# KIT-MBS/pydca

Measured on AMD Instinct MI355X. Metric: plmDCA L-BFGS iterations/s (L=500 N=50000 q=21), higher is better.
Workload: dtype f32

## Files before the change

pydca_amd/csrc/lbfgs_kernels.h:

```cpp
#pragma once

#include "dca_internal.h"
#include "plm_plan.h"
#include "vec_kernels.h"

namespace {

template <bool DD> struct DotAcc;
template <> struct DotAcc<false> {
    double hi = 0.0;
    static constexpr double lo = 0.0;
    __device__ __forceinline__ void add(double a, double b) { hi += a * b; }
    __device__ __forceinline__ void wave_reduce() { for (int off = 32; off > 0; off >>= 1) hi += __shfl_down(hi, off); }
};
template <> struct DotAcc<true> {
    double hi = 0.0, lo = 0.0;
    __device__ __forceinline__ void add(double a, double b) { dd_add(hi, lo, __dmul_rn(a, b)); }
    __device__ __forceinline__ void wave_reduce() { dd_wave_reduce(hi, lo); }
};
template <int NV>
__device__ __forceinline__ void dot_block_store(double (*red)[2 * NV], int nv, double* __restrict__ partials, unsigned grid = 0)
{
    __syncthreads();
    if ((int)threadIdx.x < nv) {
// ... 19 lines not shown
            s0.add(av, bv); s1.add(cv, cv); s2.add(av, av);
        },
        { const double av = a[i]; const double bv = b[i]; const double cv = c[i]; s0.add(av, bv); s1.add(cv, cv); s2.add(av, av); })
    s0.wave_reduce(); s1.wave_reduce(); s2.wave_reduce();
    if ((threadIdx.x & 63) == 0) {
        double* r = red[threadIdx.x >> 6];
        r[0] = s0.hi; r[1] = s0.lo; r[2] = s1.hi; r[3] = s1.lo; r[4] = s2.hi; r[5] = s2.lo;
    }
    dot_block_store<3>(red, 3, partials);
}
struct VecPtrs5 { const void* s[5]; const void* y[5]; };
struct DirCoefs { double g; double s[5]; double y[5]; };

struct LbfgsDev { double SY[5][5]; double YY[5][5]; double ys[5]; DirCoefs cf; };
constexpr int kSlotDginit = 30;

__global__ void lbfgs_two_loop_kernel(double* __restrict__ scal, LbfgsDev* __restrict__ st, int e, int endNext, int bound, double gg)
{
    if (threadIdx.x != 0 || blockIdx.x != 0) return;
    constexpr int M = 5;
    const double ys = scal[1], yy = scal[2];
    const double* G5 = scal + 3;
    double Sg[M], Yg[M], alpha[M];
    st->ys[e] = ys;
    for (int k2 = 0; k2 < M; ++k2) {
        Sg[k2] = G5[k2]; Yg[k2] = G5[5 + k2];
        st->SY[e][k2] = G5[10 + k2];
        st->SY[k2][e] = G5[15 + k2];
        st->YY[e][k2] = G5[20 + k2];
        st->YY[k2][e] = G5[20 + k2];
        alpha[k2] = 0.0;
    }
    st->SY[e][e] = ys; st->YY[e][e] = yy;
    DirCoefs cf;
    cf.g = -1.0;
    for (int k2 = 0; k2 < M; ++k2) cf.s[k2] = cf.y[k2] = 0.0;
    int j = endNext;
// ... 50 lines not shown
          const double gv = g[i]; const double sev = sev_; const double yev = yev_;
          acc[0].add(yev, sev); acc[1].add(yev, yev);
          _Pragma("unroll") for (int k = 0; k < 5; ++k) {
              const double sk = k == E ? sev : (double)static_cast<const T*>(P.s[k])[i]; const double yk = k == E ? yev : (double)static_cast<const T*>(P.y[k])[i];
              acc[2 + k].add(sk, gv); acc[7 + k].add(yk, gv); acc[12 + k].add(sev, yk); acc[17 + k].add(yev, sk); acc[22 + k].add(yev, yk);
          } })
    const int lane = threadIdx.x & 63, wv = threadIdx.x >> 6;
#pragma unroll
    for (int v = 0; v < 27; ++v) {
        acc[v].wave_reduce();
        if (lane == 0) { red[wv][2 * v] = acc[v].hi; red[wv][2 * v + 1] = acc[v].lo; }
    }
    dot_block_store<27>(red, 27, partials);
}

template <typename T>
__global__ void vec_compose_kernel(T* __restrict__ d, const T* __restrict__ g, VecPtrs5 P, const DirCoefs* __restrict__ cp, size_t n)
{
    const DirCoefs c = *cp;
    DCA_VEC_LOOP(n, d,
        const Pack<T> pg = ldp(g, iv);
        double v[VEC];
        _Pragma("unroll") for (int u = 0; u < VEC; ++u) v[u] = c.g * (double)pg.v[u];
        _Pragma("unroll") for (int k = 0; k < 5; ++k) {
            const Pack<T> psk = ldp(static_cast<const T*>(P.s[k]), iv); const Pack<T> pyk = ldp(static_cast<const T*>(P.y[k]), iv);
            _Pragma("unroll") for (int u = 0; u < VEC; ++u) v[u] += c.s[k] * (double)psk.v[u] + c.y[k] * (double)pyk.v[u];
        }
        Pack<T> o;
        _Pragma("unroll") for (int u = 0; u < VEC; ++u) o.v[u] = (T)v[u];
        stp(d, iv, o);,
        { double v = c.g * (double)g[i];
          _Pragma("unroll") for (int k = 0; k < 5; ++k)
              v += c.s[k] * (double)static_cast<const T*>(P.s[k])[i] + c.y[k] * (double)static_cast<const T*>(P.y[k])[i];
          d[i] = (T)v; })
}
#undef ldp
#undef stp

__host__ __device__ constexpr int fused_step_ti(int q, int elemBytes) { return kRowBytes / elemBytes / q; }
__host__ __device__ constexpr int fused_step_jc(int q) { return q == 21 ? 4 : 16; }
constexpr int kFusedStepThreads = 512;

template <typename T>
__device__ __forceinline__ T compose_elem(const DirCoefs& c, T gv, const T* sv, const T* yv)
{
    double v = c.g * (double)gv;
#pragma unroll
    for (int k = 0; k < 5; ++k) v += c.s[k] * (double)sv[k] + c.y[k] * (double)yv[k];
    return (T)v;
}

template <typename T, int Q>
__global__ __launch_bounds__(kFusedStepThreads)
void lbfgs_dir_trial_expand_kernel(T* __restrict__ d, T* __restrict__ xt, T* __restrict__ W, const T* __restrict__ x, const T* __restrict__ g,
                                   VecPtrs5 P, const DirCoefs* __restrict__ cp, int L, int Cs, int numJC, int pairBlocks)
// ... 9 lines not shown
    const int tid = threadIdx.x;
    const int padded = (pairBlocks + 63) / 64 * 64;
    if ((int)blockIdx.x >= padded) {
        const size_t e = (size_t)((int)blockIdx.x - padded) * kFusedStepThreads + tid;
        if (e < (size_t)L * Q) {
            T sv[5], yv[5];
#pragma unroll
            for (int k = 0; k < 5; ++k) { sv[k] = static_cast<const T*>(P.s[k])[e]; yv[k] = static_cast<const T*>(P.y[k])[e]; }
            const T dv = compose_elem(c, g[e], sv, yv);
            d[e] = dv;
            const T v = one * dv;
            xt[e] = x[e] + v;
        }
        return;
    }
    const int blk = ((int)blockIdx.x & ~63) | (((int)blockIdx.x & 7) << 3) | (((int)blockIdx.x >> 3) & 7);
    if (blk >= pairBlocks) return;
    const int i0 = (blk / numJC) * TI, j0 = (blk % numJC) * JC;
    const int j1 = min(j0 + JC, L);
    if (j1 <= i0 + 1) return;
    if (tid == 0) {
        int pre = 0;
        for (int ii = 0; ii < TI; ++ii) {
            const int i = i0 + ii, jlo = max(j0, i + 1);
            const int cnt = jlo < j1 ? (j1 - jlo) * Q2 : 0;
            const size_t before = (size_t)L * (L - 1) / 2 - (size_t)(L - i) * (L - i - 1) / 2;
            const size_t lo = cnt ? (size_t)L * Q + (before + (size_t)(jlo - i - 1)) * Q2 : 0;
            sLo[ii] = lo; sCnt[ii] = cnt; sPre[ii] = pre;
            pre += cnt ? (int)((lo + cnt + VEC - 1) / VEC - lo / VEC) : 0;
        }
        sPre[TI] = pre;
    }
    __syncthreads();
    const int total = sPre[TI];
    for (int idx = tid; idx < total; idx += kFusedStepThreads) {
// ... 81 lines not shown
{
    __shared__ double redHi[1024], redLo[1024];
    double hi = 0.0, lo = 0.0;
    for (int b = threadIdx.x; b < nA; b += blockDim.x) dd_add2(hi, lo, A[2 * (size_t)b], A[2 * (size_t)b + 1]);
    for (int b = threadIdx.x; b < nB; b += blockDim.x) dd_add2(hi, lo, B[2 * (size_t)b], B[2 * (size_t)b + 1]);
    dd_block_reduce(hi, lo, redHi, redLo);
    if (threadIdx.x == 0) out[0] = hi + lo;
}

template <typename T>
__global__ __launch_bounds__(kVecThreads)
void vec_dot3_fx_kernel(const T* __restrict__ a, const T* __restrict__ b, const T* __restrict__ c, size_t n, double* __restrict__ partials,
                        const double* __restrict__ fxParts, int nFxParts, double* __restrict__ fxChunks)
{
    if (blockIdx.x >= (unsigned)kVecBlocks) {
        __shared__ double redHi[256], redLo[256];
        const int blk = (int)blockIdx.x - kVecBlocks;
        const int chunk = (nFxParts + kSumStageBlocks - 1) / kSumStageBlocks;
        const int lo_ = blk * chunk, hi_ = min(nFxParts, lo_ + chunk);
        double hi = 0.0, lo = 0.0;
        for (int p = lo_ + threadIdx.x; p < hi_; p += blockDim.x) dd_add2(hi, lo, fxParts[2 * (size_t)p], fxParts[2 * (size_t)p + 1]);
        dd_block_reduce(hi, lo, redHi, redLo);
        if (threadIdx.x == 0) { fxChunks[2 * blk] = hi; fxChunks[2 * blk + 1] = lo; }
        return;
    }
    __shared__ double red[kVecThreads / 64][6];
    DotAcc<sizeof(T) == 8> s0, s1, s2;
    DCA_VEC_LOOP_G(n, a, kVecBlocks,
        const Pack<T> pa = ldp_at(a + head_, iv); const Pack<T> pb = ldp_at(b + head_, iv); const Pack<T> pc = ldp_at(c + head_, iv);
        _Pragma("unroll") for (int k = 0; k < VEC; ++k) {
            const double av = pa.v[k]; const double bv = pb.v[k]; const double cv = pc.v[k];
            s0.add(av, bv); s1.add(cv, cv); s2.add(av, av);
        },
        { const double av = a[i]; const double bv = b[i]; const double cv = c[i]; s0.add(av, bv); s1.add(cv, cv); s2.add(av, av); })
    s0.wave_reduce(); s1.wave_reduce(); s2.wave_reduce();
    if ((threadIdx.x & 63) == 0) {
        double* r = red[threadIdx.x >> 6];
        r[0] = s0.hi; r[1] = s0.lo; r[2] = s1.hi; r[3] = s1.lo; r[4] = s2.hi; r[5] = s2.lo;
    }
    dot_block_store<3>(red, 3, partials, kVecBlocks);
}
__global__ __launch_bounds__(1024)
void vec_final_fx_kernel(const double* __restrict__ partials, int nb, int nk, double* __restrict__ out,
                         const double* __restrict__ A, int nA, const double* __restrict__ B, int nB, double* __restrict__ fxOut)
{
    __shared__ double redHi[1024], redLo[1024];
    const int k = blockIdx.x;
    double hi = 0.0, lo = 0.0;
    if (k < nk) {
        constexpr int NT = 256;
        if ((int)threadIdx.x < NT) {
            for (int b = threadIdx.x; b < nb; b += NT) dd_add2(hi, lo, partials[2 * ((size_t)k * nb + b)], partials[2 * ((size_t)k * nb + b) + 1]);
            redHi[threadIdx.x] = hi;
            redLo[threadIdx.x] = lo;
        }
        __syncthreads();
        for (int st = NT / 2; st > 0; st >>= 1) {
            if ((int)threadIdx.x < st) dd_add2(redHi[threadIdx.x], redLo[threadIdx.x], redHi[threadIdx.x + st], redLo[threadIdx.x + st]);
            __syncthreads();
        }
        if (threadIdx.x == 0) out[k] = redHi[0] + redLo[0];
        return;
    }
    for (int b = threadIdx.x; b < nA; b += blockDim.x) dd_add2(hi, lo, A[2 * (size_t)b], A[2 * (size_t)b + 1]);
    for (int b = threadIdx.x; b < nB; b += blockDim.x) dd_add2(hi, lo, B[2 * (size_t)b], B[2 * (size_t)b + 1]);
    dd_block_reduce(hi, lo, redHi, redLo);
    if (threadIdx.x == 0) fxOut[0] = hi + lo;
}

}
```

pydca_amd/csrc/plm_engine.hip:

```cpp
#include <algorithm>
#include <chrono>
#include <cmath>

#include "dca_internal.h"
#include "more_thuente.h"
#include "vec_kernels.h"
#include "plm_plan.h"
#include "plm_stages.h"
#include "lbfgs_kernels.h"

namespace {

static_assert(kPlanXcds == kNumXcd, "the planner deals strips to this many XCDs");

#ifdef DCA_ROUND_ABLATE
__global__ void round_to_f32_kernel(double* __restrict__ p, size_t n)
{
    for (size_t i = blockIdx.x * (size_t)blockDim.x + threadIdx.x; i < n; i += (size_t)gridDim.x * blockDim.x) p[i] = (double)(float)p[i];
}
inline int round_stage_mask() { const char* e = getenv("DCA_ROUND_F32_STAGES"); return e ? atoi(e) : 0; }
#define DCA_ROUND_STAGE(bit, ptr, count)                                                                             \
    do {                                                                                                             \
        if constexpr (sizeof(T) == 8)                                                                                \
            if (round_stage_mask() & (bit))                                                                          \
// ... 40 lines not shown
    bool lbfgs_alloc = false;
    bool deferFx = false, fxPending = false;
    size_t vlo = 0, vn = 0, Ppad = 0;
    dca_comm_hook comm = nullptr;
    void* comm_user = nullptr;
    int comm_rank = 0, comm_world = 0;

    struct {
        bool begun = false, finished = false;
        int status = 0, k = 1, end = 0, iters = 0, evals = 0, max_iterations = 0, verbose = 0;
        double fx = 0, step = 0, xnorm = 0, gnorm = 0, seconds = 0;
        double last_step = 0;
        double dginit = 0;
        bool dginit_on_device = false;
        bool trial_ready = false;
    } o;

    explicit PlmEngine(dca_ctx* c) : ctx(c), N(c->N), L(c->L), q(c->q), Ls(c->Ls) {}

    template <typename U> int dalloc(U** p, size_t n)
    {
        HIP_TRY(dca_dev_malloc(reinterpret_cast<void**>(p), std::max<size_t>(n, 1) * sizeof(U)));
        return DCA_OK;
    }
    void freeall() { each_buffer([](auto*& p) { dca_dev_free(p); p = nullptr; }); }
    ~PlmEngine() override { freeall(); }

    void weights_changed() override { configured = false; o = decltype(o)(); }

    int configure(double lh, double lJ, int cmode, int chunk_, int warm_, int halo_, int add_reg_) override
// ... 30 lines not shown
        lbfgs_alloc = false;
        o = decltype(o)();

        DCA_TRY(dalloc(&dx, plan.P + kVecPad)); DCA_TRY(dalloc(&dg, plan.P + kVecPad));
        DCA_TRY(dalloc(&dWt, (size_t)plan.Wrows * plan.Cs));
        DCA_TRY(dalloc(&dSR, (size_t)N * plan.Cs));
        DCA_TRY(dalloc(&dR, (size_t)(N + kNC) * plan.Cs));
        HIP_TRY(hipMemsetAsync(dR, 0, (size_t)(N + kNC) * plan.Cs * sizeof(T), ctx->stream));
        DCA_TRY(dalloc(&dG, plan.num_slabs() * plan.slab_elems()));
        DCA_TRY(dalloc(&dw, N));
        DCA_TRY(dalloc(&dXL, (size_t)ceil_div(plan.gUnits, JT) * JT * plan.Npad));
        DCA_TRY(dalloc(&dXT2, (size_t)plan.gUnits * plan.NT));
        DCA_TRY(dalloc(&dPairs, npairs));
        DCA_TRY(dalloc(&dFxPart, 2 * (size_t)plan.nFxPart));
        DCA_TRY(dalloc(&dRegPart, 2 * (size_t)(plan.nRegPart + kSumStageBlocks)));
        DCA_TRY(dalloc(&dVecPart, 2 * 27 * kVecBlocks));
        HIP_TRY(hipMemsetAsync(dRegPart, 0, 2 * (size_t)(plan.nRegPart + kSumStageBlocks) * sizeof(double), ctx->stream));
        HIP_TRY(hipMemsetAsync(dFxPart, 0, 2 * (size_t)plan.nFxPart * sizeof(double), ctx->stream));
        if (sizeof(T) == 8) {
            DCA_TRY(dalloc(&dColPart, 2 * (size_t)kColSumRowBlocks * Lq));
            if (q == 5) DCA_TRY(dalloc(&dColChunk, 2 * (size_t)plan.numScanChunks * Lq));
            DCA_TRY(dalloc(&dColSum, (size_t)Lq));
        }
        if (strips) { DCA_TRY(dalloc(&dGrecv, plan.grecvOff[sWorld])); DCA_TRY(dalloc(&dXsend, plan.xsendOff[sWorld])); DCA_TRY(dalloc(&dXrecv, plan.xrecvOff[sWorld])); }

        HIP_TRY(hipMemsetAsync(dx, 0, (plan.P + kVecPad) * sizeof(T), ctx->stream));
        HIP_TRY(hipMemsetAsync(dg, 0, (plan.P + kVecPad) * sizeof(T), ctx->stream));
        vlo = 0; vn = plan.P; Ppad = plan.P;
        if (strips) {
            native_mode = 4;
            vlo = plan.oLo; vn = plan.oHi - plan.oLo;
// ... 219 lines not shown
                else
                    hipLaunchKernelGGL(plm_colsum_parts_kernel<T>, dim3(ceil_div(LqLoc, 64), kColSumRowBlocks), dim3(256), 0, st, dR, N, plan.Cs, LqLoc, dColPart);
                hipLaunchKernelGGL(plm_colsum_final_kernel, dim3(ceil_div(LqLoc, 256)), dim3(256), 0, st, dColPart, kColSumRowBlocks, LqLoc, dColSum);
            }
            const int nOwned = plan.pairEnd - plan.pairBegin;
            const bool mergeFields = knobs.foldMerge != 0 && !strips && nOwned > 0;
            if (!mergeFields)
            hipLaunchKernelGGL(plm_fold_fields_kernel<T>, dim3(ceil_div(LqLoc, 256)), dim3(256), 0, st, dx + (size_t)plan.cS0 * q, dG, dg + (size_t)plan.cS0 * q,
                               dRegPart + 2 * npairs, LqLoc, q, plan.Cs, (T)lambda_h, add_reg, plan.slab_elems(), foldSlabs, dColSum);
            StripMap sm;
            sm.rank = sRank; sm.world = sWorld; sm.s0 = plan.cS0; sm.s1 = plan.cS1;
            for (int r = 0; r <= sWorld; ++r) sm.site0[r] = plan.siteB[r];
            for (int r = 0; r < sWorld; ++r) { sm.recv[r] = strips && r > sRank ? dGrecv + plan.grecvOff[r] : nullptr; sm.recvCs[r] = strips ? strip_cs(r) : 0; }
            if (strips && !stripEmulate) DCA_TRY(exchange_g());
            const size_t lds = (size_t)kFoldWaves * ((q * q + 3) / 4 * 4) * sizeof(T);
            if (nOwned > 0) {
                const int pairBlocks = ceil_div(nOwned, kFoldWaves);
                FoldFieldsArgs<T> ff{dx + (size_t)plan.cS0 * q, dg + (size_t)plan.cS0 * q, dRegPart + 2 * npairs, LqLoc, (T)lambda_h, dColSum, mergeFields ? pairBlocks : -1};
                hipLaunchKernelGGL(plm_fold_pairs_kernel<T>, dim3((unsigned)(pairBlocks + (mergeFields ? ceil_div(LqLoc, 256) : 0))), dim3(64 * kFoldWaves), lds, st, dx, dG, dg, dPairs,
                                   dRegPart, L, q, plan.Cs, (T)lambda_J, add_reg, plan.slab_elems(), foldSlabs, plan.pairBegin, plan.pairEnd, sm, ff);
            }
        }
        DCA_ROUND_STAGE(16, dg, plan.P);
        fxPending = deferFx;
        if (!deferFx) {
            hipLaunchKernelGGL(dd_sum_chunks_kernel, dim3(kSumStageBlocks), dim3(256), 0, st, dRegPart, plan.nRegPart, dRegPart + 2 * (size_t)plan.nRegPart);
            hipLaunchKernelGGL(dd_sum_final_kernel, dim3(1), dim3(1024), 0, st, dRegPart + 2 * (size_t)plan.nRegPart, kSumStageBlocks, dFxPart, plan.nFxPart, ctx->dScal);
        }
        HIP_TRY(hipGetLastError());
        return DCA_OK;
    }
// ... 176 lines not shown
    }

    int gradient(double* fx_out) override
    {
        o.trial_ready = false;
        DCA_TRY(evaluate_async());
        DCA_TRY(reduce_scalars(0, 1));
        DCA_TRY(gather_vector(dg));
        DCA_TRY(read_scalars(1));
        if (fx_out) *fx_out = ctx->hScal[0];
        return DCA_OK;
    }

    void v_neg(T* d, const T* g) { hipLaunchKernelGGL(vec_neg_kernel<T>, dim3(kVecBlocks), dim3(kVecThreads), 0, ctx->stream, d + vlo, g + vlo, vn); }
    void v_step(T* x, const T* xp, double stp, const T* d) { hipLaunchKernelGGL(vec_step_kernel<T>, dim3(kVecBlocks), dim3(kVecThreads), 0, ctx->stream, x + vlo, xp + vlo, (T)stp, d + vlo, vn); }
    int eval_scalars(double* fx, double* gd, double* xx, double* gg)
    {
        if (fxPending) {
            double* const fxChunks = dRegPart + 2 * (size_t)plan.nRegPart;
            hipLaunchKernelGGL(vec_dot3_fx_kernel<T>, dim3(kVecBlocks + kSumStageBlocks), dim3(kVecThreads), 0, ctx->stream, dg + vlo, dd + vlo, dx + vlo, vn, dVecPart,
                               dRegPart, plan.nRegPart, fxChunks);
            hipLaunchKernelGGL(vec_final_fx_kernel, dim3(3 + 1), dim3(1024), 0, ctx->stream, dVecPart, kVecBlocks, 3, ctx->dScal + 1,
                               fxChunks, kSumStageBlocks, dFxPart, plan.nFxPart, ctx->dScal);
            fxPending = false;
        } else {
            hipLaunchKernelGGL(vec_dot3_kernel<T>, dim3(kVecBlocks), dim3(kVecThreads), 0, ctx->stream, dg + vlo, dd + vlo, dx + vlo, vn, dVecPart);
            hipLaunchKernelGGL(vec_final_kernel, dim3(3), dim3(256), 0, ctx->stream, dVecPart, kVecBlocks, 3, ctx->dScal + 1);
        }
        DCA_TRY(reduce_scalars(0, 4));
        DCA_TRY(read_scalars(kSlotDginit + 1));
        *fx = ctx->hScal[0]; *gd = ctx->hScal[1]; *xx = ctx->hScal[2]; *gg = ctx->hScal[3];
        if (o.dginit_on_device) { o.dginit = ctx->hScal[kSlotDginit]; o.dginit_on_device = false; }
        return DCA_OK;
    }

    int lbfgs_begin(int max_iterations, int verbose) override
    {
// ... 33 lines not shown

    int line_search(double* stp, double* f, double* xx, double* gg, int* rc_hip)
    {
        const MtParams params{1e-4, 0.9, 1e-16, 1e-20, 1e20, 5};
        const bool deferred = o.dginit_on_device;
        bool first = true;
        const int ls = mt_line_search(params, stp, f, &o.dginit, deferred, [&](double t, double* ft, double* dgt) {
            const bool ready = o.trial_ready && first && t == 1.0 && fused_step_ok();
            o.trial_ready = false; first = false;
            if (!ready) {
                v_step(dx, dxp, t, dd);
                DCA_ROUND_STAGE(32, dx, plan.P);
            }
            DCA_TRY(publish_x());
            DCA_TRY(evaluate_async(true, ready));
            return eval_scalars(ft, dgt, xx, gg);
        }, rc_hip);
        if (deferred && ls == LB_INCREASEGRADIENT) o.evals -= 1;
        return ls;
    }

    void lbfgs_end() override { o = decltype(o)(); }
    bool fused_step_ok() const
    {
#ifdef DCA_ROUND_ABLATE
        if (round_stage_mask()) return false;
#endif
        return knobs.fuseStep != 0 && native_mode == 0 && !hook && !comm && !strips && !stripEmulate && vlo == 0 && vn == plan.P &&
               plan.cS0 == 0 && plan.cS1 == L;
    }
    template <int Q> void launch_fused_step(const VecPtrs5& ptrs)
    {
        const int numJC = ceil_div(L, fused_step_jc(Q)), pairBlocks = ceil_div(L, fused_step_ti(Q, (int)sizeof(T))) * numJC;
        const size_t lds = (size_t)fused_step_ti(Q, (int)sizeof(T)) * fused_step_jc(Q) * Q * Q * sizeof(T);
        hipLaunchKernelGGL((lbfgs_dir_trial_expand_kernel<T, Q>), dim3((unsigned)(ceil_div(pairBlocks, 64) * 64 + ceil_div(L * Q, kFusedStepThreads))), dim3(kFusedStepThreads), lds,
                           ctx->stream, dd, dxp, dWt, dx, dg, ptrs, &dLb->cf, L, plan.Cs, numJC, pairBlocks);
    }
    int lbfgs_iterate(int iterations, dca_plm_stats* st) override
    {
        if (!o.begun) { dca_set_error("dca_plm_lbfgs_begin first"); return DCA_ERR_STATE; }
        auto t0 = std::chrono::steady_clock::now();
        constexpr int M = 5;
        for (int it = 0; it < iterations && !o.finished; ++it) {
            std::swap(dx, dxp);
            std::swap(dg, dgp);
// ... 10 lines not shown
            }
            o.xnorm = std::sqrt(xx); o.gnorm = std::sqrt(gg);
            o.iters = o.k;
            o.last_step = o.step;
            if (o.verbose) {
                fprintf(stderr, "Iteration %d:\n", o.k);
                fprintf(stderr, "fx = %f, xnorm = %f, gnorm = %f, step = %f\n\n", o.fx, o.xnorm, o.gnorm, o.step);
            }
            const double xn = std::max(o.xnorm, 1.0);
            if (o.gnorm / xn <= 1e-3) { o.status = 0; o.finished = true; break; }
            if (o.max_iterations != 0 && o.max_iterations < o.k + 1) { o.status = LB_MAXIMUMITERATION; o.finished = true; break; }

            const int e = o.end;
            VecPtrs5 ptrs;
            for (int i = 0; i < M; ++i) { ptrs.s[i] = dS[i] + vlo; ptrs.y[i] = dY[i] + vlo; }
            {
                ScopedKernelClock kc(ctx, "lbfgs_vec");
                auto gram = [&](auto slot) {
                    hipLaunchKernelGGL((vec_diff_gram_kernel<T, decltype(slot)::value>), dim3(kVecBlocks), dim3(kVecThreads), 0, ctx->stream, ptrs, dS[e] + vlo, dY[e] + vlo,
                                       dx + vlo, dxp + vlo, dg + vlo, dgp + vlo, vn, dVecPart);
                };
                switch (e) {
                case 0: gram(std::integral_constant<int, 0>()); break;
                case 1: gram(std::integral_constant<int, 1>()); break;
                case 2: gram(std::integral_constant<int, 2>()); break;
                case 3: gram(std::integral_constant<int, 3>()); break;
                default: gram(std::integral_constant<int, 4>()); break;
                }
                hipLaunchKernelGGL(vec_final_kernel, dim3(27), dim3(256), 0, ctx->stream, dVecPart, kVecBlocks, 27, ctx->dScal + 1);
            }
            DCA_TRY(reduce_scalars(1, 27));
            const int bound = (M <= o.k) ? M : o.k;
            ++o.k;
            o.end = (o.end + 1) % M;
            {
                ScopedKernelClock kc(ctx, "lbfgs_vec");
                hipLaunchKernelGGL(lbfgs_two_loop_kernel, dim3(1), dim3(64), 0, ctx->stream, ctx->dScal, dLb, e, o.end, bound, gg);
                if (fused_step_ok()) {
                    if (q == 21) launch_fused_step<21>(ptrs); else launch_fused_step<5>(ptrs);
                    o.trial_ready = true;
                } else {
                    hipLaunchKernelGGL(vec_compose_kernel<T>, dim3(kVecBlocks), dim3(kVecThreads), 0, ctx->stream, dd + vlo, dg + vlo, ptrs, &dLb->cf, vn);
                    DCA_ROUND_STAGE(64, dd, plan.P);
                }
                o.dginit_on_device = true;
            }
            o.step = 1.0;
        }
        HIP_TRY(hipStreamSynchronize(ctx->stream));
        o.seconds += std::chrono::duration<double>(std::chrono::steady_clock::now() - t0).count();
        if (st) {
            st->status = o.status; st->iterations = o.iters; st->evaluations = o.evals; st->finished = o.finished ? 1 : 0;
// ... 57 lines not shown
```

pydca_amd/csrc/plm_plan.h:

```cpp
#pragma once

#include <algorithm>
#include <cstddef>
#include <cstdlib>
#include <vector>

#include "../../include/dca_hip.h"

namespace {

constexpr int kPlanXcds = 8;
constexpr int kPairQ = 25;
constexpr int kNC = 128;
constexpr int kRowBytes = 512;
constexpr int kScatWavesC = 16;
constexpr int kCanonBlock = 16384;
static_assert(kCanonBlock % kNC == 0, "canonical blocks are whole tiles");
constexpr int kColSumRowBlocks = 64;
constexpr int kSumStageBlocks = 64;
constexpr int kMaxStripRanks = 64;
constexpr size_t kVecPad = 256;

struct PlmShape {
    int N = 0, L = 0, q = 0;
// ... 3 lines not shown
    int carryMode = DCA_CARRY_CHUNKED;
    int stripWorld = 1, stripRank = 0;
    bool strips = false;
};

struct PlmKnobs {
    int scatterRem = -1;
    int scatterSplit = -1;
    int scatterCanon = -1;
    int scatterWaves = -1;
    int plmPairs = -1;
    int scatterMerge = -1;
    int foldMerge = -1;
    int fuseFx = -1;
    int fuseStep = -1;
    bool is_set(int v) const { return v != -1; }
    static PlmKnobs from_env()
    {
        PlmKnobs k;
        auto rd = [](const char* name, int& v) { if (const char* e = getenv(name)) { v = atoi(e); if (v == -1) v = -2; } };
        rd("DCA_SCATTER_REM", k.scatterRem); rd("DCA_SCATTER_SPLIT", k.scatterSplit); rd("DCA_SCATTER_CANON", k.scatterCanon);
        rd("DCA_SCATTER_WAVES", k.scatterWaves); rd("DCA_PLM_PAIRS", k.plmPairs); rd("DCA_SCATTER_MERGE", k.scatterMerge);
        rd("DCA_FOLD_MERGE", k.foldMerge); rd("DCA_PLM_FUSE_FX", k.fuseFx);
        rd("DCA_PLM_FUSE_STEP", k.fuseStep);
        return k;
    }
};

struct PlmKernelShapes {
    int logitsSeqPerWg[3];
    int logitsJT[3];
    static int slot(int q) { return q == 21 ? 1 : q == kPairQ ? 2 : 0; }
};

struct ScatterLaunch {
    unsigned gridX = 0, gridY = 1;
    int N = 0, L = 0, Cs = 0, halo = 0, numChunks = 0, NT = 0, ctBase = 0, numPairs = 0, splitX = 1, numJG = 0, chunksPerSplit = 0;
    size_t slabElems = 0;
    int blockChunks = 0;
// ... 209 lines not shown
```

pydca_amd/csrc/plm_stages.h:

```cpp
#pragma once

#include "dca_internal.h"
#include "plm_plan.h"
#include "vec_kernels.h"

namespace {

#ifdef DCA_FAST_EXP
__device__ __forceinline__ float t_exp(float v) { return __expf(v); }
#else
__device__ __forceinline__ float t_exp(float v) { return expf(v); }
#endif
__device__ __forceinline__ double t_exp(double v) { return exp(v); }
__device__ __forceinline__ float t_log(float v) { return logf(v); }
__device__ __forceinline__ double t_log(double v) { return log(v); }

struct PairIJ { uint16_t i, j; };

template <typename T>
__global__ void plm_expand_kernel(const T* __restrict__ x, T* __restrict__ W, const PairIJ* __restrict__ pairs,
                                  int L, int q, int Cs, int s0, int s1)
{
    extern __shared__ __attribute__((aligned(16))) unsigned char dca_smem[];
    T* tile = reinterpret_cast<T*>(dca_smem);
// ... 633 lines not shown
    T a = G[off];
    for (int sidx = 1; sidx < nsplit; ++sidx) a += G[(size_t)sidx * slabElems + off];
    return a;
}

constexpr int kFoldWaves = 4;
struct StripMap {
    int rank = 0, world = 1, s0 = 0, s1 = 0;
    int site0[kMaxStripRanks + 1];
    const void* recv[kMaxStripRanks];
    int recvCs[kMaxStripRanks];
};
template <typename T>
__device__ __forceinline__ void fold_fields_body(const T* __restrict__ x, const T* __restrict__ G, T* __restrict__ g,
                                                 double* __restrict__ regPart, int Lq, int q, int Cs, T lambdaH, int addReg,
                                                 size_t slabElems, int nsplit, const double* __restrict__ colSum, int blk)
{
    __shared__ double red[256];
    const int c = blk * blockDim.x + threadIdx.x;
    double reg = 0.0;
    if (c < Lq) {
        const T xv = x[c];
        T gv = addReg ? (T)2 * lambdaH * xv : (T)0;
        T s = 0;
        if (colSum) s = (T)colSum[c];
        else for (int b = 0; b < q; ++b) s += slab_sum(G, (size_t)b * Cs + c, slabElems, nsplit);
        g[c] = gv + s;
        if (addReg) reg = (double)lambdaH * (double)xv * (double)xv;
    }
    __shared__ double redLo[256];
    red[threadIdx.x] = reg;
    redLo[threadIdx.x] = 0.0;
    __syncthreads();
    for (int s = blockDim.x / 2; s > 0; s >>= 1) {
        if ((int)threadIdx.x < s) dd_add2(red[threadIdx.x], redLo[threadIdx.x], red[threadIdx.x + s], redLo[threadIdx.x + s]);
        __syncthreads();
    }
    if (threadIdx.x == 0) { regPart[2 * (size_t)blk] = red[0]; regPart[2 * (size_t)blk + 1] = redLo[0]; }
}
template <typename T>
__global__ void plm_fold_fields_kernel(const T* __restrict__ x, const T* __restrict__ G, T* __restrict__ g,
                                       double* __restrict__ regPart, int Lq, int q, int Cs, T lambdaH, int addReg,
                                       size_t slabElems, int nsplit, const double* __restrict__ colSum)
{
    fold_fields_body<T>(x, G, g, regPart, Lq, q, Cs, lambdaH, addReg, slabElems, nsplit, colSum, (int)blockIdx.x);
}
template <typename T> struct FoldFieldsArgs { const T* x; T* g; double* regPart; int Lq; T lambdaH; const double* colSum; int pairBlocks; };
template <typename T>
__global__ __launch_bounds__(64 * kFoldWaves)
void plm_fold_pairs_kernel(const T* __restrict__ x, const T* __restrict__ G, T* __restrict__ g,
                           const PairIJ* __restrict__ pairs, double* __restrict__ regPart,
                           int L, int q, int Cs, T lambdaJ, int addReg, size_t slabElems, int nsplit, int pairBegin, int pairEnd,
                           const StripMap sm, const FoldFieldsArgs<T> ff)
{
    extern __shared__ __attribute__((aligned(16))) unsigned char dca_smem[];
    if (ff.pairBlocks >= 0 && (int)blockIdx.x >= ff.pairBlocks) {
        fold_fields_body<T>(ff.x, G, ff.g, ff.regPart, ff.Lq, q, Cs, ff.lambdaH, addReg, slabElems, nsplit, ff.colSum, (int)blockIdx.x - ff.pairBlocks);
        return;
    }
    const int q2 = q * q;
    const int wave = threadIdx.x >> 6, lane = threadIdx.x & 63;
    T* tile = reinterpret_cast<T*>(dca_smem) + (size_t)wave * ((q2 + 3) / 4 * 4);
    const int p = pairBegin + blockIdx.x * kFoldWaves + wave;
    if (p >= pairEnd) return;
    const int i = pairs[p].i, j = pairs[p].j;
    const int ic = (i - sm.s0) * q;
    for (int t = lane; t < q2; t += 64) {
        const int b = t / q, a = t % q;
        tile[t] = slab_sum(G, (size_t)(j * q + b) * Cs + ic + a, slabElems, nsplit);
    }
    const T* Gj = G;
    size_t jRow = (size_t)i * q, jCs = (size_t)Cs;
// ... 10 lines not shown
    const size_t base = (size_t)L * q + (size_t)p * q2;
    double reg = 0.0, regLo = 0.0;
    for (int t = lane; t < q2; t += 64) {
        const int a = t / q, b = t % q;
        const T xv = x[base + t];
        T gv = addReg ? (T)2 * lambdaJ * xv : (T)0;
        gv += tile[b * q + a];
        gv += slab_sum(Gj, (jRow + a) * jCs + jc + b, slabElems, jSplit);
        g[base + t] = gv;
        if (addReg) dd_add(reg, regLo, (double)lambdaJ * (double)xv * (double)xv);
    }
    dd_wave_reduce(reg, regLo);
    if (lane == 0) { regPart[2 * (size_t)p] = reg; regPart[2 * (size_t)p + 1] = regLo; }
}

}
```

Measured before the change: 61.42.

## Merge eval-scalar dots with L-BFGS gram pass and add tiled pair fold kernel

Adds a kernel that computes the line-search scalars (g·d, x·x, g·g) together with the s/y difference vectors and the 27 gram dots in one pass, so the two-loop update can reuse the gram results instead of rereading all vectors. It also adds an opt-in tiled fold kernel that accumulates pair couplings through LDS tiles instead of per-pair waves, and factors the tile mapping into a shared header. The merged pass removes a full memory sweep and a launch per iteration, at the cost of higher register pressure in the wider fused kernel.

```diff
diff --git a/pydca_amd/csrc/lbfgs_kernels.h b/pydca_amd/csrc/lbfgs_kernels.h
--- a/pydca_amd/csrc/lbfgs_kernels.h
+++ b/pydca_amd/csrc/lbfgs_kernels.h
@@ -2,6 +2,7 @@
 
 #include "dca_internal.h"
 #include "plm_plan.h"
+#include "plm_tiles.h"
 #include "vec_kernels.h"
 
 namespace {
@@ -57,13 +58,14 @@
 
 struct LbfgsDev { double SY[5][5]; double YY[5][5]; double ys[5]; DirCoefs cf; };
 constexpr int kSlotDginit = 30;
-
-__global__ void lbfgs_two_loop_kernel(double* __restrict__ scal, LbfgsDev* __restrict__ st, int e, int endNext, int bound, double gg)
+constexpr int kSlotGram = 32;
+
+__global__ void lbfgs_two_loop_kernel(double* __restrict__ scal, const double* __restrict__ gram, LbfgsDev* __restrict__ st, int e, int endNext, int bound, double gg)
 {
     if (threadIdx.x != 0 || blockIdx.x != 0) return;
     constexpr int M = 5;
-    const double ys = scal[1], yy = scal[2];
-    const double* G5 = scal + 3;
+    const double ys = gram[0], yy = gram[1];
+    const double* G5 = gram + 2;
     double Sg[M], Yg[M], alpha[M];
     st->ys[e] = ys;
     for (int k2 = 0; k2 < M; ++k2) {
@@ -144,6 +146,82 @@
     dot_block_store<27>(red, 27, partials);
 }
 
+__device__ __forceinline__ void fx_chunk_sum(const double* __restrict__ fxParts, int nFxParts, double* __restrict__ fxChunks, int blk)
+{
+    __shared__ double redHi[256], redLo[256];
+    const int chunk = (nFxParts + kSumStageBlocks - 1) / kSumStageBlocks;
+    const int lo_ = blk * chunk, hi_ = min(nFxParts, lo_ + chunk);
+    double hi = 0.0, lo = 0.0;
+    for (int p = lo_ + threadIdx.x; p < hi_; p += blockDim.x) dd_add2(hi, lo, fxParts[2 * (size_t)p], fxParts[2 * (size_t)p + 1]);
+    dd_block_reduce(hi, lo, redHi, redLo);
+    if (threadIdx.x == 0) { fxChunks[2 * blk] = hi; fxChunks[2 * blk + 1] = lo; }
+}
+
+constexpr int kEvalGramDots = 30;
+template <typename T, int E>
+__global__ __launch_bounds__(kVecThreads)
+void vec_eval_gram_kernel(VecPtrs5 P, T* __restrict__ se, T* __restrict__ ye, const T* __restrict__ x, const T* __restrict__ xp,
+                          const T* __restrict__ g, const T* __restrict__ gp, const T* __restrict__ d, size_t n, double* __restrict__ partials,
+                          const double* __restrict__ fxParts, int nFxParts, double* __restrict__ fxChunks)
+{
+    if (blockIdx.x >= (unsigned)kVecBlocks) {
+        fx_chunk_sum(fxParts, nFxParts, fxChunks, (int)blockIdx.x - kVecBlocks);
+        return;
+    }
+    __shared__ double red[kVecThreads / 64][2 * kEvalGramDots];
+    DotAcc<sizeof(T) == 8> ls[3];
+    DotAcc<sizeof(T) == 8> acc[27];
+    DCA_VEC_LOOP_G(n, se, kVecBlocks,
+        const Pack<T> px = ldp(x, iv); const Pack<T> pxp = ldp(xp, iv); const Pack<T> pg = ldp(g, iv); const Pack<T> pgp = ldp(gp, iv);
+        const Pack<T> pd = ldp(d, iv);
+        Pack<T> psk[5]; Pack<T> pyk[5];
+        _Pragma("unroll") for (int k = 0; k < 5; ++k)
+            if (k != E) { psk[k] = ldp(static_cast<const T*>(P.s[k]), iv); pyk[k] = ldp(static_cast<const T*>(P.y[k]), iv); }
+        Pack<T> pse; Pack<T> pye;
+        _Pragma("unroll") for (int u = 0; u < VEC; ++u) {
+            const double gv = pg.v[u]; const double dv = pd.v[u]; const double xv = px.v[u];
+            ls[0].add(gv, dv); ls[1].add(xv, xv); ls[2].add(gv, gv);
+            pse.v[u] = px.v[u] - pxp.v[u]; pye.v[u] = pg.v[u] - pgp.v[u];
+            acc[0].add((double)pye.v[u], (double)pse.v[u]); acc[1].add((double)pye.v[u], (double)pye.v[u]);
+        }
+        psk[E] = pse; pyk[E] = pye;
+        stp(se, iv, pse); stp(ye, iv, pye);
+        _Pragma("unroll") for (int k = 0; k < 5; ++k) {
+            _Pragma("unroll") for (int u = 0; u < VEC; ++u) {
+                const double gv = pg.v[u]; const double sev = pse.v[u]; const double yev = pye.v[u];
+                const double sk = psk[k].v[u]; const double yk = pyk[k].v[u];
+                acc[2 + k].add(sk, gv); acc[7 + k].add(yk, gv); acc[12 + k].add(sev, yk); acc[17 + k].add(yev, sk); acc[22 + k].add(yev, yk);
+            }
+        },
+        { const T gi = g[i]; const T xi = x[i];
+          const T sev_ = xi - xp[i]; const T yev_ = gi - gp[i];
+          const double dv = d[i];
+          double skv[5]; double ykv[5];
+          _Pragma("unroll") for (int k = 0; k < 5; ++k)
+              if (k != E) { skv[k] = (double)static_cast<const T*>(P.s[k])[i]; ykv[k] = (double)static_cast<const T*>(P.y[k])[i]; }
+          se[i] = sev_; ye[i] = yev_;
+          const double gv = gi; const double xv = xi; const double sev = sev_; const double yev = yev_;
+          skv[E] = sev; ykv[E] = yev;
+          ls[0].add(gv, dv); ls[1].add(xv, xv); ls[2].add(gv, gv);
+          acc[0].add(yev, sev); acc[1].add(yev, yev);
+          _Pragma("unroll") for (int k = 0; k < 5; ++k) {
+              const double sk = skv[k]; const double yk = ykv[k];
+              acc[2 + k].add(sk, gv); acc[7 + k].add(yk, gv); acc[12 + k].add(sev, yk); acc[17 + k].add(yev, sk); acc[22 + k].add(yev, yk);
+          } })
+    const int lane = threadIdx.x & 63, wv = threadIdx.x >> 6;
+#pragma unroll
+    for (int v = 0; v < 3; ++v) {
+        ls[v].wave_reduce();
+        if (lane == 0) { red[wv][2 * v] = ls[v].hi; red[wv][2 * v + 1] = ls[v].lo; }
+    }
+#pragma unroll
+    for (int v = 0; v < 27; ++v) {
+        acc[v].wave_reduce();
+        if (lane == 0) { red[wv][2 * (3 + v)] = acc[v].hi; red[wv][2 * (3 + v) + 1] = acc[v].lo; }
+    }
+    dot_block_store<kEvalGramDots>(red, kEvalGramDots, partials, kVecBlocks);
+}
+
 template <typename T>
 __global__ void vec_compose_kernel(T* __restrict__ d, const T* __restrict__ g, VecPtrs5 P, const DirCoefs* __restrict__ cp, size_t n)
 {
@@ -167,8 +245,6 @@
 #undef ldp
 #undef stp
 
-__host__ __device__ constexpr int fused_step_ti(int q, int elemBytes) { return kRowBytes / elemBytes / q; }
-__host__ __device__ constexpr int fused_step_jc(int q) { return q == 21 ? 4 : 16; }
 constexpr int kFusedStepThreads = 512;
 
 template <typename T>
@@ -208,11 +284,8 @@
         }
         return;
     }
-    const int blk = ((int)blockIdx.x & ~63) | (((int)blockIdx.x & 7) << 3) | (((int)blockIdx.x >> 3) & 7);
-    if (blk >= pairBlocks) return;
-    const int i0 = (blk / numJC) * TI, j0 = (blk % numJC) * JC;
-    const int j1 = min(j0 + JC, L);
-    if (j1 <= i0 + 1) return;
+    int i0, j0, j1;
+    if (!pair_tile_sites(pair_tile_deal((int)blockIdx.x), L, TI, JC, numJC, pairBlocks, i0, j0, j1)) return;
     if (tid == 0) {
         int pre = 0;
         for (int ii = 0; ii < TI; ++ii) {
@@ -324,14 +397,7 @@
                         const double* __restrict__ fxParts, int nFxParts, double* __restrict__ fxChunks)
 {
     if (blockIdx.x >= (unsigned)kVecBlocks) {
-        __shared__ double redHi[256], redLo[256];
-        const int blk = (int)blockIdx.x - kVecBlocks;
-        const int chunk = (nFxParts + kSumStageBlocks - 1) / kSumStageBlocks;
-        const int lo_ = blk * chunk, hi_ = min(nFxParts, lo_ + chunk);
-        double hi = 0.0, lo = 0.0;
-        for (int p = lo_ + threadIdx.x; p < hi_; p += blockDim.x) dd_add2(hi, lo, fxParts[2 * (size_t)p], fxParts[2 * (size_t)p + 1]);
-        dd_block_reduce(hi, lo, redHi, redLo);
-        if (threadIdx.x == 0) { fxChunks[2 * blk] = hi; fxChunks[2 * blk + 1] = lo; }
+        fx_chunk_sum(fxParts, nFxParts, fxChunks, (int)blockIdx.x - kVecBlocks);
         return;
     }
     __shared__ double red[kVecThreads / 64][6];
@@ -351,7 +417,7 @@
     dot_block_store<3>(red, 3, partials, kVecBlocks);
 }
 __global__ __launch_bounds__(1024)
-void vec_final_fx_kernel(const double* __restrict__ partials, int nb, int nk, double* __restrict__ out,
+void vec_final_fx_kernel(const double* __restrict__ partials, int nb, int nk, double* __restrict__ out, int nkLow, double* __restrict__ outHigh,
                          const double* __restrict__ A, int nA, const double* __restrict__ B, int nB, double* __restrict__ fxOut)
 {
     __shared__ double redHi[1024], redLo[1024];
@@ -369,7 +435,7 @@
             if ((int)threadIdx.x < st) dd_add2(redHi[threadIdx.x], redLo[threadIdx.x], redHi[threadIdx.x + st], redLo[threadIdx.x + st]);
             __syncthreads();
         }
-        if (threadIdx.x == 0) out[k] = redHi[0] + redLo[0];
+        if (threadIdx.x == 0) (k < nkLow ? out[k] : outHigh[k - nkLow]) = redHi[0] + redLo[0];
         return;
     }
     for (int b = threadIdx.x; b < nA; b += blockDim.x) dd_add2(hi, lo, A[2 * (size_t)b], A[2 * (size_t)b + 1]);
diff --git a/pydca_amd/csrc/plm_engine.hip b/pydca_amd/csrc/plm_engine.hip
--- a/pydca_amd/csrc/plm_engine.hip
+++ b/pydca_amd/csrc/plm_engine.hip
@@ -78,6 +78,7 @@
         double dginit = 0;
         bool dginit_on_device = false;
         bool trial_ready = false;
+        bool gram_ready = false;
     } o;
 
     explicit PlmEngine(dca_ctx* c) : ctx(c), N(c->N), L(c->L), q(c->q), Ls(c->Ls) {}
@@ -138,7 +139,7 @@
         DCA_TRY(dalloc(&dPairs, npairs));
         DCA_TRY(dalloc(&dFxPart, 2 * (size_t)plan.nFxPart));
         DCA_TRY(dalloc(&dRegPart, 2 * (size_t)(plan.nRegPart + kSumStageBlocks)));
-        DCA_TRY(dalloc(&dVecPart, 2 * 27 * kVecBlocks));
+        DCA_TRY(dalloc(&dVecPart, 2 * kEvalGramDots * kVecBlocks));
         HIP_TRY(hipMemsetAsync(dRegPart, 0, 2 * (size_t)(plan.nRegPart + kSumStageBlocks) * sizeof(double), ctx->stream));
         HIP_TRY(hipMemsetAsync(dFxPart, 0, 2 * (size_t)plan.nFxPart * sizeof(double), ctx->stream));
         if (sizeof(T) == 8) {
@@ -388,7 +389,13 @@
             for (int r = 0; r < sWorld; ++r) { sm.recv[r] = strips && r > sRank ? dGrecv + plan.grecvOff[r] : nullptr; sm.recvCs[r] = strips ? strip_cs(r) : 0; }
             if (strips && !stripEmulate) DCA_TRY(exchange_g());
             const size_t lds = (size_t)kFoldWaves * ((q * q + 3) / 4 * 4) * sizeof(T);
-            if (nOwned > 0) {
+            if (nOwned > 0 && knobs.foldTiled == 1 && plain_one_gpu()) {
+                const PairTiles pt = pair_tiles(L, Q, (int)sizeof(T));
+                const size_t ldsT = (size_t)pt.TI * pt.JC * Q * Q * sizeof(T);
+                FoldFieldsArgs<T> ff{dx, dg, dRegPart + 2 * npairs, LqLoc, (T)lambda_h, dColSum, mergeFields ? pt.pairBlocks : -1};
+                hipLaunchKernelGGL((plm_fold_tiled_kernel<T, Q>), dim3((unsigned)(pt.padded + (mergeFields ? ceil_div(LqLoc, 256) : 0))), dim3(kFoldTiledThreads), ldsT, st,
+                                   dx, dG, dg, dRegPart, L, plan.Cs, (T)lambda_J, add_reg, plan.slab_elems(), foldSlabs, pt.numJC, pt.pairBlocks, ff);
+            } else if (nOwned > 0) {
                 const int pairBlocks = ceil_div(nOwned, kFoldWaves);
                 FoldFieldsArgs<T> ff{dx + (size_t)plan.cS0 * q, dg + (size_t)plan.cS0 * q, dRegPart + 2 * npairs, LqLoc, (T)lambda_h, dColSum, mergeFields ? pairBlocks : -1};
                 hipLaunchKernelGGL(plm_fold_pairs_kernel<T>, dim3((unsigned)(pairBlocks + (mergeFields ? ceil_div(LqLoc, 256) : 0))), dim3(64 * kFoldWaves), lds, st, dx, dG, dg, dPairs,
@@ -595,13 +602,35 @@
 
     void v_neg(T* d, const T* g) { hipLaunchKernelGGL(vec_neg_kernel<T>, dim3(kVecBlocks), dim3(kVecThreads), 0, ctx->stream, d + vlo, g + vlo, vn); }
     void v_step(T* x, const T* xp, double stp, const T* d) { hipLaunchKernelGGL(vec_step_kernel<T>, dim3(kVecBlocks), dim3(kVecThreads), 0, ctx->stream, x + vlo, xp + vlo, (T)stp, d + vlo, vn); }
-    int eval_scalars(double* fx, double* gd, double* xx, double* gg)
-    {
-        if (fxPending) {
+    int eval_scalars(double* fx, double* gd, double* xx, double* gg, bool gram = false)
+    {
+        o.gram_ready = false;
+        if (fxPending && gram && merged_eval_ok()) {
+            double* const fxChunks = dRegPart + 2 * (size_t)plan.nRegPart;
+            const int e = o.end;
+            VecPtrs5 ptrs;
+            for (int i = 0; i < 5; ++i) { ptrs.s[i] = dS[i]; ptrs.y[i] = dY[i]; }
+            ScopedKernelClock kc(ctx, "lbfgs_vec");
+            auto pass = [&](auto slot) {
+                hipLaunchKernelGGL((vec_eval_gram_kernel<T, decltype(slot)::value>), dim3(kVecBlocks + kSumStageBlocks), dim3(kVecThreads), 0, ctx->stream, ptrs, dS[e], dY[e],
+                                   dx, dxp, dg, dgp, dd, plan.P, dVecPart, dRegPart, plan.nRegPart, fxChunks);
+            };
+            switch (e) {
+            case 0: pass(std::integral_constant<int, 0>()); break;
+            case 1: pass(std::integral_constant<int, 1>()); break;
+            case 2: pass(std::integral_constant<int, 2>()); break;
+            case 3: pass(std::integral_constant<int, 3>()); break;
+            default: pass(std::integral_constant<int, 4>()); break;
+            }
+            hipLaunchKernelGGL(vec_final_fx_kernel, dim3(kEvalGramDots + 1), dim3(1024), 0, ctx->stream, dVecPart, kVecBlocks, kEvalGramDots, ctx->dScal + 1, 3,
+                               ctx->dScal + kSlotGram, fxChunks, kSumStageBlocks, dFxPart, plan.nFxPart, ctx->dScal);
+            fxPending = false;
+            o.gram_ready = true;
+        } else if (fxPending) {
             double* const fxChunks = dRegPart + 2 * (size_t)plan.nRegPart;
             hipLaunchKernelGGL(vec_dot3_fx_kernel<T>, dim3(kVecBlocks + kSumStageBlocks), dim3(kVecThreads), 0, ctx->stream, dg + vlo, dd + vlo, dx + vlo, vn, dVecPart,
                                dRegPart, plan.nRegPart, fxChunks);
-            hipLaunchKernelGGL(vec_final_fx_kernel, dim3(3 + 1), dim3(1024), 0, ctx->stream, dVecPart, kVecBlocks, 3, ctx->dScal + 1,
+            hipLaunchKernelGGL(vec_final_fx_kernel, dim3(3 + 1), dim3(1024), 0, ctx->stream, dVecPart, kVecBlocks, 3, ctx->dScal + 1, 3, nullptr,
                                fxChunks, kSumStageBlocks, dFxPart, plan.nFxPart, ctx->dScal);
             fxPending = false;
         } else {
@@ -665,7 +694,7 @@
             }
             DCA_TRY(publish_x());
             DCA_TRY(evaluate_async(true, ready));
-            return eval_scalars(ft, dgt, xx, gg);
+            return eval_scalars(ft, dgt, xx, gg, true);
         }, rc_hip);
         if (deferred && ls == LB_INCREASEGRADIENT) o.evals -= 1;
         return ls;
@@ -677,9 +706,13 @@
 #ifdef DCA_ROUND_ABLATE
         if (round_stage_mask()) return false;
 #endif
-        return knobs.fuseStep != 0 && native_mode == 0 && !hook && !comm && !strips && !stripEmulate && vlo == 0 && vn == plan.P &&
-               plan.cS0 == 0 && plan.cS1 == L;
-    }
+        return knobs.fuseStep != 0 && plain_one_gpu();
+    }
+    bool plain_one_gpu() const
+    {
+        return native_mode == 0 && !hook && !comm && !strips && !stripEmulate && vlo == 0 && vn == plan.P && plan.cS0 == 0 && plan.cS1 == L;
+    }
+    bool merged_eval_ok() const { return knobs.mergeEval != 0 && knobs.fuseFx != 0 && fused_step_ok(); }
     template <int Q> void launch_fused_step(const VecPtrs5& ptrs)
     {
         const int numJC = ceil_div(L, fused_step_jc(Q)), pairBlocks = ceil_div(L, fused_step_ti(Q, (int)sizeof(T))) * numJC;
@@ -720,7 +753,9 @@
             const int e = o.end;
             VecPtrs5 ptrs;
             for (int i = 0; i < M; ++i) { ptrs.s[i] = dS[i] + vlo; ptrs.y[i] = dY[i] + vlo; }
-            {
+            const bool gramReady = o.gram_ready;
+            o.gram_ready = false;
+            if (!gramReady) {
                 ScopedKernelClock kc(ctx, "lbfgs_vec");
                 auto gram = [&](auto slot) {
                     hipLaunchKernelGGL((vec_diff_gram_kernel<T, decltype(slot)::value>), dim3(kVecBlocks), dim3(kVecThreads), 0, ctx->stream, ptrs, dS[e] + vlo, dY[e] + vlo,
@@ -741,7 +776,7 @@
             o.end = (o.end + 1) % M;
             {
                 ScopedKernelClock kc(ctx, "lbfgs_vec");
-                hipLaunchKernelGGL(lbfgs_two_loop_kernel, dim3(1), dim3(64), 0, ctx->stream, ctx->dScal, dLb, e, o.end, bound, gg);
+                hipLaunchKernelGGL(lbfgs_two_loop_kernel, dim3(1), dim3(64), 0, ctx->stream, ctx->dScal, ctx->dScal + (gramReady ? kSlotGram : 1), dLb, e, o.end, bound, gg);
                 if (fused_step_ok()) {
                     if (q == 21) launch_fused_step<21>(ptrs); else launch_fused_step<5>(ptrs);
                     o.trial_ready = true;
diff --git a/pydca_amd/csrc/plm_plan.h b/pydca_amd/csrc/plm_plan.h
--- a/pydca_amd/csrc/plm_plan.h
+++ b/pydca_amd/csrc/plm_plan.h
@@ -41,6 +41,8 @@
     int foldMerge = -1;
     int fuseFx = -1;
     int fuseStep = -1;
+    int mergeEval = -1;
+    int foldTiled = -1;
     bool is_set(int v) const { return v != -1; }
     static PlmKnobs from_env()
     {
@@ -49,7 +51,7 @@
         rd("DCA_SCATTER_REM", k.scatterRem); rd("DCA_SCATTER_SPLIT", k.scatterSplit); rd("DCA_SCATTER_CANON", k.scatterCanon);
         rd("DCA_SCATTER_WAVES", k.scatterWaves); rd("DCA_PLM_PAIRS", k.plmPairs); rd("DCA_SCATTER_MERGE", k.scatterMerge);
         rd("DCA_FOLD_MERGE", k.foldMerge); rd("DCA_PLM_FUSE_FX", k.fuseFx);
-        rd("DCA_PLM_FUSE_STEP", k.fuseStep);
+        rd("DCA_PLM_FUSE_STEP", k.fuseStep); rd("DCA_PLM_MERGE_EVAL", k.mergeEval); rd("DCA_FOLD_TILED", k.foldTiled);
         return k;
     }
 };
diff --git a/pydca_amd/csrc/plm_stages.h b/pydca_amd/csrc/plm_stages.h
--- a/pydca_amd/csrc/plm_stages.h
+++ b/pydca_amd/csrc/plm_stages.h
@@ -2,6 +2,7 @@
 
 #include "dca_internal.h"
 #include "plm_plan.h"
+#include "plm_tiles.h"
 #include "vec_kernels.h"
 
 namespace {
@@ -671,12 +672,13 @@
 template <typename T>
 __device__ __forceinline__ void fold_fields_body(const T* __restrict__ x, const T* __restrict__ G, T* __restrict__ g,
                                                  double* __restrict__ regPart, int Lq, int q, int Cs, T lambdaH, int addReg,
-                                                 size_t slabElems, int nsplit, const double* __restrict__ colSum, int blk)
+                                                 size_t slabElems, int nsplit, const double* __restrict__ colSum, int blk, int nt)
 {
     __shared__ double red[256];
-    const int c = blk * blockDim.x + threadIdx.x;
+    const bool on = (int)threadIdx.x < nt;
+    const int c = blk * nt + threadIdx.x;
     double reg = 0.0;
-    if (c < Lq) {
+    if (on && c < Lq) {
         const T xv = x[c];
         T gv = addReg ? (T)2 * lambdaH * xv : (T)0;
         T s = 0;
@@ -686,10 +688,9 @@
         if (addReg) reg = (double)lambdaH * (double)xv * (double)xv;
     }
     __shared__ double redLo[256];
-    red[threadIdx.x] = reg;
-    redLo[threadIdx.x] = 0.0;
+    if (on) { red[threadIdx.x] = reg; redLo[threadIdx.x] = 0.0; }
     __syncthreads();
-    for (int s = blockDim.x / 2; s > 0; s >>= 1) {
+    for (int s = nt / 2; s > 0; s >>= 1) {
         if ((int)threadIdx.x < s) dd_add2(red[threadIdx.x], redLo[threadIdx.x], red[threadIdx.x + s], redLo[threadIdx.x + s]);
         __syncthreads();
     }
@@ -700,7 +701,7 @@
                                        double* __restrict__ regPart, int Lq, int q, int Cs, T lambdaH, int addReg,
                                        size_t slabElems, int nsplit, const double* __restrict__ colSum)
 {
-    fold_fields_body<T>(x, G, g, regPart, Lq, q, Cs, lambdaH, addReg, slabElems, nsplit, colSum, (int)blockIdx.x);
+    fold_fields_body<T>(x, G, g, regPart, Lq, q, Cs, lambdaH, addReg, slabElems, nsplit, colSum, (int)blockIdx.x, (int)blockDim.x);
 }
 template <typename T> struct FoldFieldsArgs { const T* x; T* g; double* regPart; int Lq; T lambdaH; const double* colSum; int pairBlocks; };
 template <typename T>
@@ -712,7 +713,7 @@
 {
     extern __shared__ __attribute__((aligned(16))) unsigned char dca_smem[];
     if (ff.pairBlocks >= 0 && (int)blockIdx.x >= ff.pairBlocks) {
-        fold_fields_body<T>(ff.x, G, ff.g, ff.regPart, ff.Lq, q, Cs, ff.lambdaH, addReg, slabElems, nsplit, ff.colSum, (int)blockIdx.x - ff.pairBlocks);
+        fold_fields_body<T>(ff.x, G, ff.g, ff.regPart, ff.Lq, q, Cs, ff.lambdaH, addReg, slabElems, nsplit, ff.colSum, (int)blockIdx.x - ff.pairBlocks, (int)blockDim.x);
         return;
     }
     const int q2 = q * q;
@@ -753,4 +754,86 @@
     if (lane == 0) { regPart[2 * (size_t)p] = reg; regPart[2 * (size_t)p + 1] = regLo; }
 }
 
-}
+constexpr int kFoldTiledThreads = 512;
+template <typename T, int Q>
+__global__ __launch_bounds__(kFoldTiledThreads)
+void plm_fold_tiled_kernel(const T* __restrict__ x, const T* __restrict__ G, T* __restrict__ g, double* __restrict__ regPart,
+                           int L, int Cs, T lambdaJ, int addReg, size_t slabElems, int nsplit, int numJC, int pairBlocks,
+                           const FoldFieldsArgs<T> ff)
+{
+    constexpr int TI = fused_step_ti(Q, (int)sizeof(T)), JC = fused_step_jc(Q), Q2 = Q * Q;
+    extern __shared__ __attribute__((aligned(16))) unsigned char dca_smem[];
+    T* tile = reinterpret_cast<T*>(dca_smem);
+    const int tid = threadIdx.x;
+    const int padded = (pairBlocks + 63) / 64 * 64;
+    if ((int)blockIdx.x >= padded) {
+        if (ff.pairBlocks >= 0)
+            fold_fields_body<T>(ff.x, G, ff.g, ff.regPart, ff.Lq, Q, Cs, ff.lambdaH, addReg, slabElems, nsplit, ff.colSum, (int)blockIdx.x - padded, 256);
+        return;
+    }
+    int i0, j0, j1;
+    if (!pair_tile_sites(pair_tile_deal((int)blockIdx.x), L, TI, JC, numJC, pairBlocks, i0, j0, j1)) return;
+    {
+        const int wave = tid >> 6, lane = tid & 63;
+        for (int pp = wave; pp < TI * JC; pp += kFoldTiledThreads / 64) {
+            const int i = i0 + pp / JC, j = j0 + pp % JC;
+            if (j <= i || j >= j1) continue;
+            const size_t p = pair_index(L, i, j);
+            const size_t base = (size_t)L * Q + p * Q2;
+            T* const tl = tile + (size_t)pp * Q2;
+            double reg = 0.0, regLo = 0.0;
+            for (int t = lane; t < Q2; t += 64) {
+                const T xv = x[base + t];
+                tl[t] = addReg ? (T)2 * lambdaJ * xv : (T)0;
+                if (addReg) dd_add(reg, regLo, (double)lambdaJ * (double)xv * (double)xv);
+            }
+            dd_wave_reduce(reg, regLo);
+            if (lane == 0) { regPart[2 * p] = reg; regPart[2 * p + 1] = regLo; }
+        }
+    }
+    __syncthreads();
+    auto phases = [&](auto oneSlab) {
+        constexpr bool ONE = decltype(oneSlab)::value;
+        {
+            constexpr int WD = TI * Q, NEL = JC * Q * WD;
+#pragma unroll
+            for (int k = 0; k < (NEL + kFoldTiledThreads - 1) / kFoldTiledThreads; ++k) {
+                const int idx = tid + k * kFoldTiledThreads;
+                const int row = idx / WD, col = idx % WD;
+                const int jj = row / Q, ii = col / Q;
+                const int i = i0 + ii, j = j0 + jj;
+                if (idx < NEL && j > i && j < j1) {
+                    const size_t off = (size_t)(j0 * Q + row) * Cs + i0 * Q + col;
+                    tile[col * Q + ii * ((JC - 1) * Q2) + row + jj * ((Q - 1) * Q)] += ONE ? G[off] : slab_sum(G, off, slabElems, nsplit);
+                }
+            }
+        }
+        __syncthreads();
+        {
+            constexpr int WD = JC * Q, NEL = TI * Q * WD;
+#pragma unroll
+            for (int k = 0; k < (NEL + kFoldTiledThreads - 1) / kFoldTiledThreads; ++k) {
+                const int idx = tid + k * kFoldTiledThreads;
+                const int row = idx / WD, col = idx % WD;
+                const int ii = row / Q, jj = col / Q;
+                const int i = i0 + ii, j = j0 + jj;
+                if (idx < NEL && j > i && j < j1) {
+                    const size_t off = (size_t)(i0 * Q + row) * Cs + j0 * Q + col;
+                    tile[row * Q + ii * ((JC - 1) * Q2) + col + jj * ((Q - 1) * Q)] += ONE ? G[off] : slab_sum(G, off, slabElems, nsplit);
+                }
+            }
+        }
+        __syncthreads();
+    };
+    if (nsplit == 1) phases(std::true_type()); else phases(std::false_type());
+    for (int ii = 0; ii < TI; ++ii) {
+        const int i = i0 + ii, jlo = max(j0, i + 1);
+        if (jlo >= j1) continue;
+        const int cnt = (j1 - jlo) * Q2;
+        T* const dst = g + (size_t)L * Q + pair_index(L, i, jlo) * Q2;
+        const T* const src = tile + (size_t)(ii * JC + (jlo - j0)) * Q2;
+        for (int t = tid; t < cnt; t += kFoldTiledThreads) dst[t] = src[t];
+    }
+}
+
+}
diff --git a/pydca_amd/csrc/plm_tiles.h b/pydca_amd/csrc/plm_tiles.h
--- /dev/null
+++ b/pydca_amd/csrc/plm_tiles.h
@@ -0,0 +1,37 @@
+#pragma once
+
+#include "plm_plan.h"
+
+#ifdef __HIPCC__
+#define DCA_TILE_HD __host__ __device__
+#else
+#define DCA_TILE_HD
+#endif
+
+namespace {
+
+DCA_TILE_HD constexpr int fused_step_ti(int q, int elemBytes) { return kRowBytes / elemBytes / q; }
+DCA_TILE_HD constexpr int fused_step_jc(int q) { return q == 21 ? 4 : 16; }
+
+struct PairTiles {
+    int TI, JC, numJC, pairBlocks, padded;
+};
+DCA_TILE_HD inline PairTiles pair_tiles(int L, int q, int elemBytes)
+{
+    PairTiles t;
+    t.TI = fused_step_ti(q, elemBytes); t.JC = fused_step_jc(q);
+    t.numJC = (L + t.JC - 1) / t.JC;
+    t.pairBlocks = (L + t.TI - 1) / t.TI * t.numJC;
+    t.padded = (t.pairBlocks + 63) / 64 * 64;
+    return t;
+}
+DCA_TILE_HD inline int pair_tile_deal(int wg) { return (wg & ~63) | ((wg & 7) << 3) | ((wg >> 3) & 7); }
+DCA_TILE_HD inline bool pair_tile_sites(int blk, int L, int TI, int JC, int numJC, int pairBlocks, int& i0, int& j0, int& j1)
+{
+    if (blk >= pairBlocks) return false;
+    i0 = (blk / numJC) * TI; j0 = (blk % numJC) * JC;
+    j1 = j0 + JC < L ? j0 + JC : L;
+    return j1 > i0 + 1;
+}
+
+}
```

New measurement: 61.99, median of 6. Within noise of the previous version (+0.9%).
